# JitongZ/shockwave-replication

Hardware: AMD Instinct MI355X
Metric: Shockwave plan solves/sec at 900 jobs x 30 rounds (higher is better)
Workload: dtype f64 objective / fp32 ranking keys

## Files before the change

shockwave-replication_amd/csrc/sw_api.hip:

```cpp
#include <hip/hip_runtime.h>
#include <stdint.h>
#include <string.h>

#include <stdlib.h>

#include <algorithm>
#include <atomic>
#include <climits>
#include <new>
#include <string>
#include <thread>
#include <vector>

#include "../../include/shockwave_amd.h"
#include "sw_arith.h"
#include "sw_device.h"
#include "sw_handle.h"
#include "sw_p2x.h"
#include "sw_validate.h"

static int fuse_max_count() {
    static const int v = [] {
        const char* e = getenv("SW_FUSE_MAX");
        return e ? atoi(e) : 256;
    }();
    return v;
}

static int split_min_count() {
    static const int v = [] {
        const char* e = getenv("SW_SPLIT_MIN");
        return e ? atoi(e) : 256;
    }();
    return v;
}


extern "C" size_t sw_plan_kernel_lds_bytes(int one);
extern "C" hipError_t sw_launch_plan(const sw_batch_dev* B, int KT, int one, size_t lds,
                                     hipStream_t stream);
extern "C" hipError_t sw_launch_split(sw_batch_dev* B, size_t p2x_lds, hipStream_t stream);
extern "C" hipError_t sw_launch_p2x(const sw_batch_dev* B, int maxN, int maxT, hipStream_t stream);
extern "C" size_t sw_p2x_kernel_lds_bytes(int maxN, int maxT);

namespace {

thread_local std::string g_create_error;

}

namespace {
// ... 102 lines not shown
    }
    h->ev_pool.assign(2 * kEventPairs, nullptr);
    h->ev_p2x.assign(2 * kEventPairs, nullptr);
    for (size_t i = 0; e == hipSuccess && i < h->ev_pool.size(); ++i) e = hipEventCreate(&h->ev_pool[i]);
    for (size_t i = 0; e == hipSuccess && i < h->ev_p2x.size(); ++i) e = hipEventCreate(&h->ev_p2x[i]);
    if (e != hipSuccess) {
        g_create_error = std::string("HIP init failed: ") + hipGetErrorString(e);
        sw_destroy(h);
        return nullptr;
    }
    if (cfg && cfg->max_instances > 0 && cfg->max_total_jobs > 0) {
        size_t J = (size_t)cfg->max_total_jobs, I = (size_t)cfg->max_instances;
        if (h->d_in.reserve(in_block_bytes((int32_t)I, (int64_t)J)) ||
            h->d_res.reserve(res_block_bytes((int32_t)I, (int64_t)J, (int64_t)J * SW_MAX_ROUNDS)) ||
            h->d_masks.reserve(J) || h->d_nb.reserve(J) || h->d_lvl.reserve(I) ||
            h->d_p2ws.reserve(J * SW_P2X_ARR_BYTES) ||
            h->h_in.reserve(in_block_bytes((int32_t)I, (int64_t)J)) ||
            h->h_res.reserve(res_block_bytes((int32_t)I, (int64_t)J, (int64_t)J * SW_MAX_ROUNDS)) ||
            h->h_masks.reserve(J)) {
            g_create_error = "device reservation failed";
            sw_destroy(h);
            return nullptr;
        }
    }
    return h;
}

void sw_destroy(sw_handle* h) {
    if (!h) return;
    (void)hipSetDevice(h->device);
    if (h->stream) (void)hipStreamSynchronize(h->stream);
    if (h->up) (void)hipStreamSynchronize(h->up);
    if (h->dn) (void)hipStreamSynchronize(h->dn);
    sw_shard_release(h);
    sw_mmf_release(h);
    h->d_in.release(); h->d_res.release();
    h->d_ws_u8.release(); h->d_ws_u64.release(); h->d_ws_sort.release();
    h->d_ws_keys.release(); h->d_ws_jc.release(); h->d_stamps.release();
    h->d_masks.release(); h->d_p2ws.release(); h->d_nb.release(); h->d_lvl.release();
    h->h_in.release(); h->h_res.release();
    h->h_masks.release();
    for (hipEvent_t ev : h->ev_chunk)
        if (ev) (void)hipEventDestroy(ev);
    if (h->up) (void)hipStreamDestroy(h->up);
    if (h->dn) (void)hipStreamDestroy(h->dn);
    for (hipEvent_t ev : h->ev_xs)
        if (ev) (void)hipEventDestroy(ev);
    for (hipStream_t x : h->xs)
        if (x) (void)hipStreamDestroy(x);
    for (hipEvent_t ev : h->ev_pool)
        if (ev) (void)hipEventDestroy(ev);
    for (hipEvent_t ev : h->ev_p2x)
        if (ev) (void)hipEventDestroy(ev);
    if (h->own_stream && h->stream) (void)hipStreamDestroy(h->stream);
// ... 67 lines not shown
        P += (int64_t)pr.num_jobs * pr.future_rounds;
        maxN = std::max(maxN, pr.num_jobs);
        maxT = std::max(maxT, pr.future_rounds);
    }
    SW_HIP(h, hipStreamSynchronize(h->stream));
    if (h->up) SW_HIP(h, hipStreamSynchronize(h->up));
    if (h->dn) SW_HIP(h, hipStreamSynchronize(h->dn));
    if (collect_timing(h) != SW_OK) return SW_ERR_HIP;
    h->loaded = false;
    h->count = 0;
    h->total_jobs = 0;
    h->total_plan = 0;
    const size_t Jz = (size_t)std::max<int64_t>(J, 1);
    const size_t inb = in_block_bytes(std::max(count, 1), (int64_t)Jz), resb = res_block_bytes(std::max(count, 1), (int64_t)Jz, std::max<int64_t>(P, 1));
    if (h->d_in.reserve(inb) || h->d_res.reserve(resb) ||
        h->d_masks.reserve(Jz) || h->d_nb.reserve(Jz) || h->d_lvl.reserve(std::max(count, 1)))
        return fail(h, SW_ERR_HIP, "device allocation failed");
    if (maxN > SW_LDS_JOBS || maxT > 32) {
        const int KT = maxT <= 32 ? 32 : 64;
        if (h->d_ws_u8.reserve(Jz * SW_WS_U8) || h->d_ws_u64.reserve(Jz * SW_WS_U64 + (size_t)SW_WS_PAD_U64 * std::max(count, 1)) ||
            h->d_ws_sort.reserve(Jz * 4) || h->d_ws_keys.reserve(Jz * KT) ||
            h->d_ws_jc.reserve(Jz))
            return fail(h, SW_ERR_HIP, "workspace allocation failed");
    }
    if (h->d_p2ws.reserve(Jz * SW_P2X_ARR_BYTES))
        return fail(h, SW_ERR_HIP, "P2 exchange workspace allocation failed");
    if (h->h_in.reserve(inb) || h->h_res.reserve(resb) || h->h_masks.reserve(Jz))
        return fail(h, SW_ERR_HIP, "pinned allocation failed");
    set_views(h, std::max(count, 1), (int64_t)Jz, std::max<int64_t>(P, 1));
    h->inst.resize(count);
    h->Ns.resize(count);
// ... 109 lines not shown
    B.inst = h->d_inst + lo;
    B.count = hi - lo;
    B.KT = h->maxT <= 32 ? 32 : 64;
    B.w = h->d_w;
    B.d = h->d_d;
    B.F = h->d_F;
    B.E = h->d_E;
    B.R = h->d_R;
    B.p = h->d_p;
    B.plan = h->d_plan;
    B.planned = h->d_planned;
    B.masks = h->d_masks.p;
    B.out = h->d_out + lo;
    B.nb = h->d_nb.p;
    B.lvl = h->d_lvl.p + lo;
#ifdef SW_STAMPS
    B.stamps = h->d_stamps.p + (size_t)lo * SW_STAMP_SLOTS;
#endif
    const int one = h->maxN <= SW_LDS_JOBS && h->maxT <= 32;
    if (!one) {
        B.ws.u8 = h->d_ws_u8.p;
        B.ws.u64 = h->d_ws_u64.p;
        B.ws.sort = h->d_ws_sort.p;
        B.ws.keys = h->d_ws_keys.p;
        B.ws.jc = h->d_ws_jc.p;
    }
    B.p2ws = h->d_p2ws.p;
    size_t lds = sw_plan_kernel_lds_bytes(one);
    if (timed) {
        if (h->ev_used == kEventPairs && collect_timing(h) != SW_OK) return SW_ERR_HIP;
        SW_HIP(h, hipEventRecord(h->ev_pool[2 * h->ev_used], s));
    }
#ifdef SW_STAMPS
    const bool split = false;
#else
    const bool split = one && (force_split >= 0 ? force_split != 0 : B.count > split_min_count());
#endif
    B.fuse_p2x = one && (split || B.count <= fuse_max_count());
    if (B.fuse_p2x) lds = std::max(lds, sw_p2x_kernel_lds_bytes(h->maxN, h->maxT));
    hipError_t e = split ? sw_launch_split(&B, sw_p2x_kernel_lds_bytes(h->maxN, h->maxT), s)
                         : sw_launch_plan(&B, B.KT, one, lds, s);
    if (e != hipSuccess) return hip_fail(h, e, "plan kernel launch");
    if (timed) {
        SW_HIP(h, hipEventRecord(h->ev_pool[2 * h->ev_used + 1], s));
        SW_HIP(h, hipEventRecord(h->ev_p2x[2 * h->ev_used], s));
    }
    if (!B.fuse_p2x) {
        e = sw_launch_p2x(&B, h->maxN, h->maxT, s);
        if (e != hipSuccess) return hip_fail(h, e, "sw_p2x_kernel launch");
    }
    if (timed) {
        SW_HIP(h, hipEventRecord(h->ev_p2x[2 * h->ev_used + 1], s));
        h->ev_used++;
// ... 120 lines not shown
    static const int req = [] {
        const char* e = getenv("SW_RUN_STREAMS");
        return e ? atoi(e) : -1;
    }();
#ifdef SW_STAMPS
    return 1;
#endif
    const bool one = h->maxN <= SW_LDS_JOBS && h->maxT <= 32;
    if (!one || h->count <= split_min_count()) return 1;
    int ns = req >= 0 ? req : (h->count <= 2048 ? 2 : 1);
    ns = std::max(1, std::min(ns, kMaxRunStreams));
    return std::min(ns, std::max(1, h->count / 64));
}

int launch_streams(sw_handle* h, int ns) {
    if (h->xs.empty()) {
        h->xs.assign(kMaxRunStreams - 1, nullptr);
        h->ev_xs.assign(kMaxRunStreams, nullptr);
        for (auto& x : h->xs) SW_HIP(h, hipStreamCreateWithFlags(&x, hipStreamNonBlocking));
        for (auto& ev : h->ev_xs) SW_HIP(h, hipEventCreateWithFlags(&ev, hipEventDisableTiming));
    }
    const bool timed = h->timing;
    if (timed) {
        if (h->ev_used == kEventPairs && collect_timing(h) != SW_OK) return SW_ERR_HIP;
        SW_HIP(h, hipEventRecord(h->ev_pool[2 * h->ev_used], h->stream));
    }
    SW_HIP(h, hipEventRecord(h->ev_xs[0], h->stream));
    for (int c = 1; c < ns; ++c) SW_HIP(h, hipStreamWaitEvent(h->xs[c - 1], h->ev_xs[0], 0));
    int err = SW_OK;
    for (int c = 0; c < ns && err == SW_OK; ++c) {
        const int32_t lo = (int32_t)((int64_t)h->count * c / ns), hi = (int32_t)((int64_t)h->count * (c + 1) / ns);
        err = launch(h, lo, hi, c == 0 ? h->stream : h->xs[c - 1], false, h->keep_masks, 1);
    }
    for (int c = 1; c < ns; ++c) {
        SW_HIP(h, hipEventRecord(h->ev_xs[c], h->xs[c - 1]));
// ... 130 lines not shown
```

shockwave-replication_amd/csrc/sw_device.h:

```cpp
#pragma once
#include <stdint.h>

#include "sw_arith.h"

#define SW_STAMP_SLOTS 64
#define SW_LDS_JOBS 1024

struct sw_inst_dev {
    int32_t N, T, G, nb;
    int64_t job_off;
    int64_t plan_off;
    double delta, k;
    double beta[SW_BMAX];
    double ell[SW_BMAX];
};

struct sw_out_dev {
    double objective, utility, makespan, p2_objective, bound;
    int32_t iters, status;
};

struct sw_ws_dev {
    uint8_t* u8;
    uint64_t* u64;
// ... 21 lines not shown
    const int32_t* E;
    const double* R;
    const double* p;
    uint8_t* plan;
    int32_t* planned;
    uint64_t* masks;
    sw_out_dev* out;
    uint8_t* nb;
    sw_lvl_dev* lvl;
    int32_t only_slow;
    sw_ws_dev ws;
    unsigned char* p2ws;
    int32_t fuse_p2x;
    int32_t want_masks;
    int32_t lds_bytes;
    uint64_t* stamps;
};
```

shockwave-replication_amd/csrc/sw_handle.h:

```cpp
#pragma once
#include <hip/hip_runtime.h>
#include <stdint.h>

#include <algorithm>
#include <string>
#include <vector>

#include "../../include/shockwave_amd.h"
#include "sw_device.h"

struct sw_shard_state;

template <typename T>
struct DevBuf {
    T* p = nullptr;
    size_t cap = 0;
    hipError_t reserve(size_t n) {
        if (n <= cap) return hipSuccess;
        if (p) (void)hipFree(p);
        p = nullptr;
        cap = 0;
        size_t want = std::max<size_t>(n, 1);
        hipError_t e = hipMalloc((void**)&p, want * sizeof(T));
        if (e == hipSuccess) cap = want;
// ... 43 lines not shown
    std::vector<int32_t> Ns, Ts;
    sw_inst_dev* d_inst = nullptr;
    DevBuf<unsigned char> d_in, d_res;
    int32_t *d_w = nullptr, *d_F = nullptr, *d_E = nullptr, *d_planned = nullptr;
    double *d_d = nullptr, *d_R = nullptr, *d_p = nullptr;
    uint8_t* d_plan = nullptr;
    sw_out_dev* d_out = nullptr;
    size_t in_bytes = 0, res_bytes = 0;
    DevBuf<uint8_t> d_ws_u8;
    DevBuf<uint64_t> d_ws_u64, d_ws_sort;
    DevBuf<float> d_ws_keys;
    DevBuf<sw_jobc> d_ws_jc;
    DevBuf<uint64_t> d_masks;
    DevBuf<uint8_t> d_nb;
    DevBuf<sw_lvl_dev> d_lvl;
    DevBuf<unsigned char> d_p2ws;
    DevBuf<uint64_t> d_stamps;
    HostBuf<unsigned char> h_in, h_res;
    int32_t *h_w = nullptr, *h_F = nullptr, *h_E = nullptr, *h_planned = nullptr;
    double *h_d = nullptr, *h_R = nullptr, *h_p = nullptr;
    uint8_t* h_plan = nullptr;
    sw_out_dev* h_out = nullptr;
    HostBuf<uint64_t> h_masks;
    sw_inst_dev* h_inst = nullptr;
    hipStream_t up = nullptr, dn = nullptr;
    std::vector<hipEvent_t> ev_chunk;
    std::vector<hipStream_t> xs;
    std::vector<hipEvent_t> ev_xs;
    int32_t pend_count = 0;
    int64_t pend_jobs = 0, pend_plan = 0;
// ... 14 lines not shown
```

shockwave-replication_amd/csrc/sw_kernels.hip:

```cpp
#include <hip/hip_runtime.h>
#include <stdint.h>

#include "../../include/shockwave_amd.h"
#include "sw_arith.h"
#include "sw_block.h"
#include "sw_device.h"
#include "sw_pack.h"
#include "sw_bnb.h"
#include "sw_repair.h"
#include "sw_reround_dev.h"
#include "sw_p2x_inst.h"

namespace {

#ifdef SW_STAMPS
#define SW_STAMP(slot)                                                            \
    do {                                                                          \
        __syncthreads();                                                          \
        if (threadIdx.x == 0 && B.stamps) {                                       \
            uint64_t now_ = __builtin_amdgcn_s_memtime();                         \
            B.stamps[(size_t)inst_ * SW_STAMP_SLOTS + (slot)] += now_ - stamp_prev_;      \
            stamp_prev_ = now_;                                                   \
        }                                                                         \
    } while (0)
// ... 76 lines not shown
    double inv_delta;
    int64_t passes;
    double lsU, lsM;
    const sw_inst_dev* inst;
    const double* beta;
    const double* ell;
    const double* slope;
    sw_blk blk;
    const int32_t* w_in;
    const double* p_in;
#ifdef SW_STAMPS
    uint64_t* swp;
    uint64_t* lsp;
    uint64_t ls_t;
    uint64_t lsa[9];
#endif
    uint8_t *ncur, *lcur, *tkcur, *nbest, *placed, *placed2, *nfin;
    uint8_t* tiecur;
    uint64_t *ycur, *ybest, *y2;
    uint32_t* pst;
    uint64_t* pmask;
    int32_t* pord;
    uint64_t* sbuf;
    int32_t *H, *SH;
    sw_pack_lds* PL;
    int32_t pwc;
    int32_t* caps;
    int64_t* misc;
    sw_repair_t* rep;
    sw_bnb_ivl* bnb;
// ... 770 lines not shown
                k2 = 0;
            } else if (MODE != 2 && MODE != 5) {
                const double lvl = gval(j, s, nj - 1);
                const bool crit = k > 0.0 && lvl > Mb;
                k1 = crit ? (SW_CRIT_BIT | sw_bits(lvl)) : (MODE == 3 ? (uint64_t)jc(j, s).w : 0);
                k2 = kbits(j, s, nj - 1);
            } else {
                k1 = sw_ratio_key(p_in[j] / (double)nj);
                k2 = 0;
            }
            khi = k1;
            klo = ((uint64_t)k2 << 32) | (uint64_t)(0xFFFFFFFFu - (uint32_t)j);
        }
    }

    __device__ __forceinline__ void pack(int MODE, const uint8_t* nin, uint64_t* y,
                                         uint8_t* placed_out) {
        __syncthreads();
#ifdef SW_STAMPS
        uint64_t pk0_ = __builtin_amdgcn_s_memtime();
#define PK_STAMP(k)                                                      \
    do {                                                                 \
        const uint64_t n_ = __builtin_amdgcn_s_memtime();                \
        if (threadIdx.x == 0 && swp) swp[40 + (k)] += n_ - pk0_;         \
        pk0_ = n_;                                                       \
    } while (0)
#else
#define PK_STAMP(k) \
    do {            \
    } while (0)
#endif
        double Mb = 0.0;
        const int32_t* capsp = MODE == 5 ? caps : nullptr;
        if (MODE == 1 || MODE == 3) {
            for_jobs([&](int j, int s) { Mb = sw_max(Mb, gval(j, s, nin[j])); });
            Mb = blk.dmax(Mb);
        }
        int64_t act_l = 0;
        if constexpr (ONE) {
            constexpr int E = SW_JPT;
            uint64_t khi[E], klo[E];
#pragma unroll
            for (int s = 0; s < E; ++s) { khi[s] = 0; klo[s] = 0; }
            for_jobs([&](int j, int s) {
                key_of(MODE, nin, Mb, j, s, khi[s], klo[s]);
                act_l += nin_of(MODE, nin, j) > 0;
                if (owns(MODE, nin, j)) y[j] = 0;
            });
            int32_t A32;
            const int32_t abase = blk.exscan((int32_t)act_l, A32);
            const int A_ = A32;
            PK_STAMP(0);
#ifdef SW_STAMPS
            const uint64_t srt0_ = __builtin_amdgcn_s_memtime();
#endif
            const bool ratio = MODE == 2 || MODE == 4 || MODE == 5;
            if (ratio) {
#pragma unroll
                for (int s = 0; s < E; ++s)
                    khi[s] = khi[s] != 0 || klo[s] != 0
                                 ? (khi[s] << 11) | (uint64_t)(2047u - (0xFFFFFFFFu - (uint32_t)klo[s]))
                                 : 0ull;
            }
            if (SMALL || A_ <= SW_BLOCK) {
                uint64_t* xh = sbuf;
                uint64_t* xl = sbuf + SW_BLOCK;
                int b = abase;
#pragma unroll
                for (int s = 0; s < E; ++s)
                    if (klo[s] != 0) {
                        xh[b] = khi[s];
                        if constexpr (!SMALL) xl[b] = klo[s];
                        ++b;
                    }
                __syncthreads();
                const bool mine = (int)threadIdx.x < A_;
                uint64_t h1 = mine ? xh[threadIdx.x] : 0ull;
                uint64_t l1 = 0ull;
                if constexpr (SMALL) {
                    sort_one<false>(h1, l1, sbuf + SW_BLOCK);
                } else {
                    l1 = mine ? xl[threadIdx.x] : 0ull;
                    if (ratio) sort_one<false>(h1, l1, sbuf + 2 * SW_BLOCK);
                    else sort_one<true>(h1, l1, sbuf + 2 * SW_BLOCK);
                }
#ifdef SW_STAMPS
                if (threadIdx.x == 0 && swp) swp[7] += __builtin_amdgcn_s_memtime() - srt0_;
                pk0_ = __builtin_amdgcn_s_memtime();
#endif
                const int jp1 = !mine ? 0
                                : ratio ? (int)(2047u - (uint32_t)(h1 & 2047u))
                                        : (int)(0xFFFFFFFFu - (uint32_t)(l1 & 0xFFFFFFFFu));
                const uint32_t wq = MODE == 5 ? 1u : (uint32_t)w_in[jp1];
                uint32_t st1[1] = {mine ? ((uint32_t)nin[jp1] | (wq << 8)) : 0u};
                uint64_t mk1[1] = {0ull};
                PK_STAMP(1);
#ifdef SW_STAMPS
                sw_pack_rounds_one<SMALL>(PL, A_, T, G, st1[0], mk1[0], sbuf, capsp, swp);
#else
                sw_pack_rounds_one<SMALL>(PL, A_, T, G, st1[0], mk1[0], sbuf, capsp);
#endif
                PK_STAMP(2);
                for_jobs([&](int j, int s) {
                    (void)s;
                    if (owns(MODE, nin, j)) placed_out[j] = 0;
                });
                __syncthreads();
                if (mine) {
                    y[jp1] = mk1[0];
                    placed_out[jp1] = (uint8_t)(nin[jp1] - st_r(st1[0]));
                }
                __syncthreads();
                PK_STAMP(3);
            } else {
                if constexpr (!SMALL) {
                if (ratio) sort_regs64(khi);
                else sort_regs(khi, klo);
#ifdef SW_STAMPS
                if (threadIdx.x == 0 && swp) swp[7] += __builtin_amdgcn_s_memtime() - srt0_;
#endif
                uint32_t st[E];
                uint64_t mk[E];
                int jp[E];
#pragma unroll
                for (int s = 0; s < E; ++s) {
                    const int p = E * (int)threadIdx.x + s;
                    mk[s] = 0;
                    jp[s] = ratio ? (int)(2047u - (uint32_t)(khi[s] & 2047u))
                                  : (int)(0xFFFFFFFFu - (uint32_t)(klo[s] & 0xFFFFFFFFu));
                    const uint32_t wq = MODE == 5 ? 1u : (uint32_t)w_in[jp[s]];
                    st[s] = (p < A_) ? ((uint32_t)nin[jp[s]] | (wq << 8)) : 0u;
                }
#ifdef SW_STAMPS
                sw_pack_rounds<SW_JPT>(blk, PL, A_, T, G, st, mk, capsp, swp);
// ... 5 lines not shown
                    if (owns(MODE, nin, j)) placed_out[j] = 0;
                });
                __syncthreads();
#pragma unroll
                for (int s = 0; s < E; ++s) {
                    const int p = E * (int)threadIdx.x + s;
                    if (p < A_) {
                        y[jp[s]] = mk[s];
                        placed_out[jp[s]] = (uint8_t)(nin[jp[s]] - st_r(st[s]));
                    }
                }
                __syncthreads();
                            }
            }
        } else {
            int NPg = 1;
            while (NPg < N) NPg <<= 1;
            uint64_t* shi = sbuf;
            uint64_t* slo = sbuf + NPg;
            for (int i = threadIdx.x; i < NPg; i += SW_BLOCK) { shi[i] = 0; slo[i] = 0; }
            __syncthreads();
            for (int j = jlo(); j < jhi(); ++j) {
                uint64_t khi, klo;
                key_of(MODE, nin, Mb, j, 0, khi, klo);
                shi[j] = khi;
                slo[j] = klo;
                act_l += nin_of(MODE, nin, j) > 0;
                if (owns(MODE, nin, j)) y[j] = 0;
            }
            const int A_ = (int)blk.sum(act_l);
// ... 8 lines not shown
            }
            __syncthreads();
            if (wave_id() == 0) rounds(A_, PPL, capsp);
            __syncthreads();
            for (int j = jlo(); j < jhi(); ++j)
                if (owns(MODE, nin, j)) placed_out[j] = 0;
            __syncthreads();
            for (int p = threadIdx.x; p < A_; p += SW_BLOCK) {
                const int s = tslot(p, PPL);
                const int j = pord[s];
                y[j] = pmask[s];
                placed_out[j] = (uint8_t)(nin[j] - st_r(pst[s]));
            }
            __syncthreads();
        }
#undef PK_STAMP
    }

    __device__ __forceinline__ bool repair_pack(const uint8_t* nin, const uint64_t* yd,
                                                const uint8_t* pd, uint64_t* yout, uint8_t* pout) {
        sw_repair_t* R = rep;
        uint32_t* wset = reinterpret_cast<uint32_t*>(misc);
        int32_t* flag = reinterpret_cast<int32_t*>(misc) + 8;
        __syncthreads();
        for (int i = threadIdx.x; i < (int)(sizeof(sw_repair_t) / 4); i += SW_BLOCK)
            reinterpret_cast<int32_t*>(R)[i] = 0;
        if (threadIdx.x < 8) wset[threadIdx.x] = 0;
        __syncthreads();
        for_jobs([&](int j, int s) {
            (void)s;
            if (nin[j] > 0) atomicOr(&wset[(w_in[j] >> 5) & 7], 1u << (w_in[j] & 31));
        });
// ... 230 lines not shown
    if (one) {
        const size_t NJ = SW_LDS_JOBS;
        s += 8 * r16(NJ) + 3 * r16(8 * NJ) + r16(8 * 4 * SW_JPT * SW_BLOCK) + SW_JOB_LDS_BYTES;
    } else {
        s += 2 * r16(8 * (SW_RR_CAPMAX + 1)) + r16(8 * SW_RR_WORDS);
    }
    return s;
}

__host__ __device__ constexpr size_t sw_level_lds_bytes() {
    auto r16 = [](size_t b) { return (b + 15) & ~(size_t)15; };
    return r16(sizeof(sw_xchg)) + r16(sizeof(double) * 3 * SW_BMAX) +
           r16(sizeof(float) * SW_JPT * SW_SETUP_CH * SW_BLOCK) + SW_JOB_LDS_BYTES;
}

__host__ __device__ constexpr size_t sw_pack_lds_bytes() {
    auto r16 = [](size_t b) { return (b + 15) & ~(size_t)15; };
    const size_t NJ = SW_LDS_JOBS;
    return r16(sizeof(sw_xchg)) + r16(sizeof(sw_pack_lds)) + r16(sizeof(int64_t) * 8) +
           r16(sizeof(sw_repair_t)) + 3 * r16(NJ) + 2 * r16(8 * NJ) + r16(8 * 3 * SW_BLOCK);
}

template <int KT>
__device__ __forceinline__ void level_instance(const sw_batch_dev& B, unsigned char* smem, int inst_) {
    const sw_inst_dev* I = &B.inst[inst_];
    Ctx<KT, true> c;
    c.inst = I;
    c.N = I->N;
    c.T = I->T;
    c.G = I->G;
    c.nb = I->nb;
    c.C = (int64_t)I->G * I->T;
    c.k = I->k;
    c.inv_delta = 1.0 / I->delta;
    c.passes = 0;
// ... 92 lines not shown
        uint64_t m = ym[j];
        uint32_t wv[4] = {0u, 0u, 0u, 0u};
#pragma unroll
        for (int k = 0; k < 16; ++k) {
            wv[k >> 2] |= (uint32_t)((m >> t) & 1ull) << ((k & 3) * 8);
            if (++t == T) {
                t = 0;
                ++j;
                if (k < 15 && j < N) m = ym[j];
            }
        }
        dst[ci] = make_uint4(wv[0], wv[1], wv[2], wv[3]);
    }
}

__device__ __forceinline__ const uint64_t* pack_instance(const sw_batch_dev& B, unsigned char* smem, int inst_) {
    const sw_inst_dev* I = &B.inst[inst_];
    Ctx<32, true, true> c;
    c.inst = I;
    c.N = I->N;
    c.T = I->T;
    c.G = I->G;
    c.nb = I->nb;
    c.C = (int64_t)I->G * I->T;
    c.k = I->k;
    c.inv_delta = 1.0 / I->delta;
    const sw_lvl_dev lv = B.lvl[inst_];
    c.passes = lv.passes;
    c.q = (c.N + SW_BLOCK - 1) / SW_BLOCK;
    const int64_t jo = I->job_off;
    c.w_in = B.w + jo;
    c.p_in = B.p + jo;
#ifdef SW_STAMPS
    c.swp = nullptr;
    c.lsp = nullptr;
#endif
    size_t off = 0;
    auto carve = [&](size_t bytes) {
        unsigned char* p = smem + off;
        off += (bytes + 15) & ~(size_t)15;
        return p;
    };
    c.blk.X = (sw_xchg*)carve(sizeof(sw_xchg));
    c.blk.par = 0;
    c.beta = c.ell = c.slope = nullptr;
    c.PL = (sw_pack_lds*)carve(sizeof(sw_pack_lds));
    c.H = c.PL->H[0];
    c.SH = c.PL->SH[0];
    c.caps = c.PL->H[1];
    c.pwc = 0;
    c.misc = (int64_t*)carve(sizeof(int64_t) * 8);
    c.rep = (sw_repair_t*)carve(sizeof(sw_repair_t));
    const int NJ = SW_LDS_JOBS;
    c.nbest = carve(NJ);
    c.placed = carve(NJ);
    c.placed2 = carve(NJ);
    c.ncur = c.lcur = c.tkcur = c.nfin = c.tiecur = nullptr;
    c.bnb = nullptr;
    c.ycur = (uint64_t*)carve(sizeof(uint64_t) * NJ);
    c.y2 = (uint64_t*)carve(sizeof(uint64_t) * NJ);
    c.ybest = nullptr;
    c.sbuf = (uint64_t*)carve(sizeof(uint64_t) * 3 * SW_BLOCK);
    c.pst = nullptr;
    c.pord = nullptr;
    c.pmask = nullptr;
    c.gkeys = nullptr;
    c.gjc = nullptr;
    if (off != sw_pack_lds_bytes()) __builtin_trap();
    int64_t act_l = 0;
    c.for_jobs([&](int j, int s) {
        (void)s;
        c.nbest[j] = B.nb[jo + j];
        act_l += c.nbest[j] > 0;
    });
    sw_out_dev* out = &B.out[inst_];
    if (c.blk.sum(act_l) > SW_BLOCK) {
        if (threadIdx.x == 0) out->status = SW_STATUS_SLOW_MARK;
        return nullptr;
    }
    c.pack(4, c.nbest, c.ycur, c.placed);
    int64_t def_l = 0;
    c.for_jobs([&](int j, int s) {
        (void)s;
        def_l += (int64_t)c.w_in[j] * (c.nbest[j] - c.placed[j]);
    });
    int64_t dfc = c.blk.sum(def_l);
    c.passes++;
    int32_t status = 0;
    if (dfc != 0 && c.repair_pack(c.nbest, c.ycur, c.placed, c.y2, c.placed2)) {
        c.for_jobs([&](int j, int s) {
            (void)s;
            c.ycur[j] = c.y2[j];
        });
        c.passes++;
        dfc = 0;
// ... 44 lines not shown
                                          int inst) {
    const sw_inst_dev* I = &B.inst[inst];
    sw_out_dev* out = &B.out[inst];
    const int N = I->N, T = I->T, G = I->G;
    const int64_t jo = I->job_off;
    const int q = (N + SW_BLOCK - 1) / SW_BLOCK;
    const int j0 = sw_tid_opaque() * q, j1 = min(j0 + q, N);
    __syncthreads();
    int act = 0;
#pragma unroll
    for (int k = 0; k < 2; ++k) act += (j0 + k < j1 && ym[j0 + k] != 0ull) ? 1 : 0;
    const bool run = B.fuse_p2x && !(out->status & SW_STATUS_P2_FALLBACK);
    sw_p2x_lds* L = reinterpret_cast<sw_p2x_lds*>(smem);
    const size_t Lsz = (sizeof(sw_p2x_lds) + 15) & ~(size_t)15;
    unsigned char* var = smem + Lsz;
    sw_blk blk;
    blk.X = &L->X;
    blk.par = 0;
    int A = 0;
    const int a0 = blk.exscan(act, A);
    A = __builtin_amdgcn_readfirstlane(A);
    const uint64_t* yemit = ym;
    if (run && A > 0 && A <= SW_P2X_AMAX) {
        const size_t vb = (sw_p2x_var_bytes(A, T) + 15) & ~(size_t)15;
        const bool onchip = Lsz + vb + (size_t)SW_P2X_ARR_BYTES * A <= (size_t)B.lds_bytes &&
                            var + vb >= reinterpret_cast<const unsigned char*>(ym + N);
        unsigned char* base = onchip ? var + vb : B.p2ws + (size_t)SW_P2X_ARR_BYTES * jo;
        const size_t n = onchip ? (size_t)A : (size_t)N;
        sw_p2x_arrays X;
        X.cc = reinterpret_cast<double*>(base);
// ... 598 lines not shown
        if (B.fuse_p2x) {
            __syncthreads();
            sw_p2x_instance(B, B.p2ws, sw_smem, blockIdx.x);
        }
    }
}

template <int KT>
__global__ __launch_bounds__(SW_BLOCK, 4) void sw_level_kernel(sw_batch_dev B) {
    extern __shared__ __attribute__((aligned(16))) unsigned char sw_smem[];
    level_instance<KT>(B, sw_smem, blockIdx.x);
}

__global__ __launch_bounds__(SW_BLOCK, 8) void sw_pack_kernel(sw_batch_dev B) {
    extern __shared__ __attribute__((aligned(16))) unsigned char sw_smem[];
    const uint64_t* ym = pack_instance(B, sw_smem, blockIdx.x);
    if (ym) pack_tail(B, ym, sw_smem, blockIdx.x);
}

extern "C" size_t sw_plan_kernel_lds_bytes(int one) { return sw_plan_lds_bytes(one != 0); }

extern "C" hipError_t sw_launch_split(sw_batch_dev* B, size_t p2x_lds, hipStream_t stream) {
    dim3 grid(B->count), block(SW_BLOCK);
    B->only_slow = 0;
    B->fuse_p2x = 1;
    hipLaunchKernelGGL((sw_level_kernel<32>), grid, block, sw_level_lds_bytes(), stream, *B);
    B->lds_bytes = (int32_t)std::max(sw_pack_lds_bytes(), p2x_lds);
    hipLaunchKernelGGL(sw_pack_kernel, grid, block, (size_t)B->lds_bytes, stream, *B);
    B->only_slow = 1;
    hipLaunchKernelGGL((sw_plan_kernel<32, true>), grid, block, std::max(sw_plan_lds_bytes(true), p2x_lds),
                       stream, *B);
    B->only_slow = 0;
    return hipGetLastError();
}

extern "C" hipError_t sw_launch_plan(const sw_batch_dev* B, int KT, int one, size_t lds,
                                     hipStream_t stream) {
    dim3 grid(B->count), block(SW_BLOCK);
    if (KT == 32) {
        if (one) hipLaunchKernelGGL((sw_plan_kernel<32, true>), grid, block, lds, stream, *B);
        else hipLaunchKernelGGL((sw_plan_kernel<32, false>), grid, block, lds, stream, *B);
    } else {
        hipLaunchKernelGGL((sw_plan_kernel<64, false>), grid, block, lds, stream, *B);
// ... 4 lines not shown
```

Measured before the change: 2.549 million.

## Split pack stage into sort, wave-per-instance rounds, and place kernels

For large split batches (count at or above SW_LOOP_MIN, default 4096), the fused pack kernel is broken into three launches. A sort kernel writes ranked job words to global workspace. A rounds kernel runs the round-packing loop with one wave per instance, four instances per block. A place kernel reads the results back and runs the pack tail. The aim is to stop a whole block waiting on the serial rounds loop, at the cost of extra launches and global round-trips. Stream and event creation in launch_streams also becomes lazy, sized to the requested count.

Result: faster. 2.768 million, median of 6 (+8.6%).

```diff
diff --git a/shockwave-replication_amd/csrc/sw_api.hip b/shockwave-replication_amd/csrc/sw_api.hip
--- a/shockwave-replication_amd/csrc/sw_api.hip
+++ b/shockwave-replication_amd/csrc/sw_api.hip
@@ -35,6 +35,13 @@
     return v;
 }
 
+static int loop_min_count() {
+    static const int v = [] {
+        const char* e = getenv("SW_LOOP_MIN");
+        return e ? atoi(e) : 4096;
+    }();
+    return v;
+}
 
 extern "C" size_t sw_plan_kernel_lds_bytes(int one);
 extern "C" hipError_t sw_launch_plan(const sw_batch_dev* B, int KT, int one, size_t lds,
@@ -167,6 +174,7 @@
         if (h->d_in.reserve(in_block_bytes((int32_t)I, (int64_t)J)) ||
             h->d_res.reserve(res_block_bytes((int32_t)I, (int64_t)J, (int64_t)J * SW_MAX_ROUNDS)) ||
             h->d_masks.reserve(J) || h->d_nb.reserve(J) || h->d_lvl.reserve(I) ||
+            h->d_lws.reserve(J) || h->d_lwm.reserve(J) || h->d_lwa.reserve(I) ||
             h->d_p2ws.reserve(J * SW_P2X_ARR_BYTES) ||
             h->h_in.reserve(in_block_bytes((int32_t)I, (int64_t)J)) ||
             h->h_res.reserve(res_block_bytes((int32_t)I, (int64_t)J, (int64_t)J * SW_MAX_ROUNDS)) ||
@@ -191,6 +199,7 @@
     h->d_ws_u8.release(); h->d_ws_u64.release(); h->d_ws_sort.release();
     h->d_ws_keys.release(); h->d_ws_jc.release(); h->d_stamps.release();
     h->d_masks.release(); h->d_p2ws.release(); h->d_nb.release(); h->d_lvl.release();
+    h->d_lws.release(); h->d_lwm.release(); h->d_lwa.release();
     h->h_in.release(); h->h_res.release();
     h->h_masks.release();
     for (hipEvent_t ev : h->ev_chunk)
@@ -288,7 +297,8 @@
     const size_t Jz = (size_t)std::max<int64_t>(J, 1);
     const size_t inb = in_block_bytes(std::max(count, 1), (int64_t)Jz), resb = res_block_bytes(std::max(count, 1), (int64_t)Jz, std::max<int64_t>(P, 1));
     if (h->d_in.reserve(inb) || h->d_res.reserve(resb) ||
-        h->d_masks.reserve(Jz) || h->d_nb.reserve(Jz) || h->d_lvl.reserve(std::max(count, 1)))
+        h->d_masks.reserve(Jz) || h->d_nb.reserve(Jz) || h->d_lvl.reserve(std::max(count, 1)) ||
+        h->d_lws.reserve(Jz) || h->d_lwm.reserve(Jz) || h->d_lwa.reserve(std::max(count, 1)))
         return fail(h, SW_ERR_HIP, "device allocation failed");
     if (maxN > SW_LDS_JOBS || maxT > 32) {
         const int KT = maxT <= 32 ? 32 : 64;
@@ -428,6 +438,9 @@
     B.out = h->d_out + lo;
     B.nb = h->d_nb.p;
     B.lvl = h->d_lvl.p + lo;
+    B.lws = h->d_lws.p;
+    B.lwm = h->d_lwm.p;
+    B.lwa = h->d_lwa.p + lo;
 #ifdef SW_STAMPS
     B.stamps = h->d_stamps.p + (size_t)lo * SW_STAMP_SLOTS;
 #endif
@@ -451,6 +464,7 @@
     const bool split = one && (force_split >= 0 ? force_split != 0 : B.count > split_min_count());
 #endif
     B.fuse_p2x = one && (split || B.count <= fuse_max_count());
+    B.loop_split = split && B.count >= loop_min_count();
     if (B.fuse_p2x) lds = std::max(lds, sw_p2x_kernel_lds_bytes(h->maxN, h->maxT));
     hipError_t e = split ? sw_launch_split(&B, sw_p2x_kernel_lds_bytes(h->maxN, h->maxT), s)
                          : sw_launch_plan(&B, B.KT, one, lds, s);
@@ -601,11 +615,15 @@
 }
 
 int launch_streams(sw_handle* h, int ns) {
-    if (h->xs.empty()) {
-        h->xs.assign(kMaxRunStreams - 1, nullptr);
-        h->ev_xs.assign(kMaxRunStreams, nullptr);
-        for (auto& x : h->xs) SW_HIP(h, hipStreamCreateWithFlags(&x, hipStreamNonBlocking));
-        for (auto& ev : h->ev_xs) SW_HIP(h, hipEventCreateWithFlags(&ev, hipEventDisableTiming));
+    while ((int)h->xs.size() < ns - 1) {
+        hipStream_t x = nullptr;
+        SW_HIP(h, hipStreamCreateWithFlags(&x, hipStreamNonBlocking));
+        h->xs.push_back(x);
+    }
+    while ((int)h->ev_xs.size() < ns) {
+        hipEvent_t ev = nullptr;
+        SW_HIP(h, hipEventCreateWithFlags(&ev, hipEventDisableTiming));
+        h->ev_xs.push_back(ev);
     }
     const bool timed = h->timing;
     if (timed) {
diff --git a/shockwave-replication_amd/csrc/sw_device.h b/shockwave-replication_amd/csrc/sw_device.h
--- a/shockwave-replication_amd/csrc/sw_device.h
+++ b/shockwave-replication_amd/csrc/sw_device.h
@@ -59,5 +59,9 @@
     int32_t fuse_p2x;
     int32_t want_masks;
     int32_t lds_bytes;
+    int32_t loop_split;
+    uint32_t* lws;
+    uint64_t* lwm;
+    int32_t* lwa;
     uint64_t* stamps;
 };
diff --git a/shockwave-replication_amd/csrc/sw_handle.h b/shockwave-replication_amd/csrc/sw_handle.h
--- a/shockwave-replication_amd/csrc/sw_handle.h
+++ b/shockwave-replication_amd/csrc/sw_handle.h
@@ -81,6 +81,9 @@
     DevBuf<uint64_t> d_masks;
     DevBuf<uint8_t> d_nb;
     DevBuf<sw_lvl_dev> d_lvl;
+    DevBuf<uint32_t> d_lws;
+    DevBuf<uint64_t> d_lwm;
+    DevBuf<int32_t> d_lwa;
     DevBuf<unsigned char> d_p2ws;
     DevBuf<uint64_t> d_stamps;
     HostBuf<unsigned char> h_in, h_res;
diff --git a/shockwave-replication_amd/csrc/sw_kernels.hip b/shockwave-replication_amd/csrc/sw_kernels.hip
--- a/shockwave-replication_amd/csrc/sw_kernels.hip
+++ b/shockwave-replication_amd/csrc/sw_kernels.hip
@@ -114,6 +114,7 @@
     uint64_t* lsp;
     uint64_t ls_t;
     uint64_t lsa[9];
+    uint64_t pk0_, srt0;
 #endif
     uint8_t *ncur, *lcur, *tkcur, *nbest, *placed, *placed2, *nfin;
     uint8_t* tiecur;
@@ -914,11 +915,7 @@
         }
     }
 
-    __device__ __forceinline__ void pack(int MODE, const uint8_t* nin, uint64_t* y,
-                                         uint8_t* placed_out) {
-        __syncthreads();
 #ifdef SW_STAMPS
-        uint64_t pk0_ = __builtin_amdgcn_s_memtime();
 #define PK_STAMP(k)                                                      \
     do {                                                                 \
         const uint64_t n_ = __builtin_amdgcn_s_memtime();                \
@@ -930,94 +927,127 @@
     do {            \
     } while (0)
 #endif
+
+    template <bool ZY = true>
+    __device__ __forceinline__ bool pack_front(int MODE, const uint8_t* nin, uint64_t* y,
+                                               uint64_t (&khi)[SW_JPT], uint64_t (&klo)[SW_JPT], int& A_,
+                                               bool& mine, int& jp1, uint32_t& st1) {
+        constexpr int E = SW_JPT;
         double Mb = 0.0;
-        const int32_t* capsp = MODE == 5 ? caps : nullptr;
         if (MODE == 1 || MODE == 3) {
             for_jobs([&](int j, int s) { Mb = sw_max(Mb, gval(j, s, nin[j])); });
             Mb = blk.dmax(Mb);
         }
         int64_t act_l = 0;
+#pragma unroll
+        for (int s = 0; s < E; ++s) { khi[s] = 0; klo[s] = 0; }
+        for_jobs([&](int j, int s) {
+            key_of(MODE, nin, Mb, j, s, khi[s], klo[s]);
+            act_l += nin_of(MODE, nin, j) > 0;
+            if constexpr (ZY)
+                if (owns(MODE, nin, j)) y[j] = 0;
+        });
+        int32_t A32;
+        const int32_t abase = blk.exscan((int32_t)act_l, A32);
+        A_ = A32;
+        PK_STAMP(0);
+#ifdef SW_STAMPS
+        const uint64_t srt0_ = __builtin_amdgcn_s_memtime();
+        srt0 = srt0_;
+#endif
+        const bool ratio = MODE == 2 || MODE == 4 || MODE == 5;
+        if (ratio) {
+#pragma unroll
+            for (int s = 0; s < E; ++s)
+                khi[s] = khi[s] != 0 || klo[s] != 0
+                             ? (khi[s] << 11) | (uint64_t)(2047u - (0xFFFFFFFFu - (uint32_t)klo[s]))
+                             : 0ull;
+        }
+        if (!(SMALL || A_ <= SW_BLOCK)) return false;
+        uint64_t* xh = sbuf;
+        uint64_t* xl = sbuf + SW_BLOCK;
+        int b = abase;
+#pragma unroll
+        for (int s = 0; s < E; ++s)
+            if (klo[s] != 0) {
+                xh[b] = khi[s];
+                if constexpr (!SMALL) xl[b] = klo[s];
+                ++b;
+            }
+        __syncthreads();
+        mine = (int)threadIdx.x < A_;
+        uint64_t h1 = mine ? xh[threadIdx.x] : 0ull;
+        uint64_t l1 = 0ull;
+        if constexpr (SMALL) {
+            sort_one<false>(h1, l1, sbuf + SW_BLOCK);
+        } else {
+            l1 = mine ? xl[threadIdx.x] : 0ull;
+            if (ratio) sort_one<false>(h1, l1, sbuf + 2 * SW_BLOCK);
+            else sort_one<true>(h1, l1, sbuf + 2 * SW_BLOCK);
+        }
+#ifdef SW_STAMPS
+        if (threadIdx.x == 0 && swp) swp[7] += __builtin_amdgcn_s_memtime() - srt0_;
+        pk0_ = __builtin_amdgcn_s_memtime();
+#endif
+        jp1 = !mine ? 0
+              : ratio ? (int)(2047u - (uint32_t)(h1 & 2047u))
+                      : (int)(0xFFFFFFFFu - (uint32_t)(l1 & 0xFFFFFFFFu));
+        const uint32_t wq = MODE == 5 ? 1u : (uint32_t)w_in[jp1];
+        st1 = mine ? ((uint32_t)nin[jp1] | (wq << 8)) : 0u;
+        PK_STAMP(1);
+        return true;
+    }
+
+    __device__ __forceinline__ void pack_loop(int MODE, int A_, uint32_t& st1, uint64_t& mk1) {
+        const int32_t* capsp = MODE == 5 ? caps : nullptr;
+#ifdef SW_STAMPS
+        sw_pack_rounds_one<SMALL>(PL, A_, T, G, st1, mk1, sbuf, capsp, swp);
+#else
+        sw_pack_rounds_one<SMALL>(PL, A_, T, G, st1, mk1, sbuf, capsp);
+#endif
+        PK_STAMP(2);
+    }
+
+    __device__ __forceinline__ void pack_back(int MODE, const uint8_t* nin, uint64_t* y,
+                                              uint8_t* placed_out, bool mine, int jp1, uint32_t st1,
+                                              uint64_t mk1) {
+        for_jobs([&](int j, int s) {
+            (void)s;
+            if (owns(MODE, nin, j)) placed_out[j] = 0;
+        });
+        __syncthreads();
+        if (mine) {
+            y[jp1] = mk1;
+            placed_out[jp1] = (uint8_t)(nin[jp1] - st_r(st1));
+        }
+        __syncthreads();
+        PK_STAMP(3);
+    }
+
+    __device__ __forceinline__ void pack(int MODE, const uint8_t* nin, uint64_t* y,
+                                         uint8_t* placed_out) {
+        __syncthreads();
+#ifdef SW_STAMPS
+        pk0_ = __builtin_amdgcn_s_memtime();
+#endif
+        const int32_t* capsp = MODE == 5 ? caps : nullptr;
         if constexpr (ONE) {
             constexpr int E = SW_JPT;
             uint64_t khi[E], klo[E];
-#pragma unroll
-            for (int s = 0; s < E; ++s) { khi[s] = 0; klo[s] = 0; }
-            for_jobs([&](int j, int s) {
-                key_of(MODE, nin, Mb, j, s, khi[s], klo[s]);
-                act_l += nin_of(MODE, nin, j) > 0;
-                if (owns(MODE, nin, j)) y[j] = 0;
-            });
-            int32_t A32;
-            const int32_t abase = blk.exscan((int32_t)act_l, A32);
-            const int A_ = A32;
-            PK_STAMP(0);
-#ifdef SW_STAMPS
-            const uint64_t srt0_ = __builtin_amdgcn_s_memtime();
-#endif
-            const bool ratio = MODE == 2 || MODE == 4 || MODE == 5;
-            if (ratio) {
-#pragma unroll
-                for (int s = 0; s < E; ++s)
-                    khi[s] = khi[s] != 0 || klo[s] != 0
-                                 ? (khi[s] << 11) | (uint64_t)(2047u - (0xFFFFFFFFu - (uint32_t)klo[s]))
-                                 : 0ull;
-            }
-            if (SMALL || A_ <= SW_BLOCK) {
-                uint64_t* xh = sbuf;
-                uint64_t* xl = sbuf + SW_BLOCK;
-                int b = abase;
-#pragma unroll
-                for (int s = 0; s < E; ++s)
-                    if (klo[s] != 0) {
-                        xh[b] = khi[s];
-                        if constexpr (!SMALL) xl[b] = klo[s];
-                        ++b;
-                    }
-                __syncthreads();
-                const bool mine = (int)threadIdx.x < A_;
-                uint64_t h1 = mine ? xh[threadIdx.x] : 0ull;
-                uint64_t l1 = 0ull;
-                if constexpr (SMALL) {
-                    sort_one<false>(h1, l1, sbuf + SW_BLOCK);
-                } else {
-                    l1 = mine ? xl[threadIdx.x] : 0ull;
-                    if (ratio) sort_one<false>(h1, l1, sbuf + 2 * SW_BLOCK);
-                    else sort_one<true>(h1, l1, sbuf + 2 * SW_BLOCK);
-                }
-#ifdef SW_STAMPS
-                if (threadIdx.x == 0 && swp) swp[7] += __builtin_amdgcn_s_memtime() - srt0_;
-                pk0_ = __builtin_amdgcn_s_memtime();
-#endif
-                const int jp1 = !mine ? 0
-                                : ratio ? (int)(2047u - (uint32_t)(h1 & 2047u))
-                                        : (int)(0xFFFFFFFFu - (uint32_t)(l1 & 0xFFFFFFFFu));
-                const uint32_t wq = MODE == 5 ? 1u : (uint32_t)w_in[jp1];
-                uint32_t st1[1] = {mine ? ((uint32_t)nin[jp1] | (wq << 8)) : 0u};
-                uint64_t mk1[1] = {0ull};
-                PK_STAMP(1);
-#ifdef SW_STAMPS
-                sw_pack_rounds_one<SMALL>(PL, A_, T, G, st1[0], mk1[0], sbuf, capsp, swp);
-#else
-                sw_pack_rounds_one<SMALL>(PL, A_, T, G, st1[0], mk1[0], sbuf, capsp);
-#endif
-                PK_STAMP(2);
-                for_jobs([&](int j, int s) {
-                    (void)s;
-                    if (owns(MODE, nin, j)) placed_out[j] = 0;
-                });
-                __syncthreads();
-                if (mine) {
-                    y[jp1] = mk1[0];
-                    placed_out[jp1] = (uint8_t)(nin[jp1] - st_r(st1[0]));
-                }
-                __syncthreads();
-                PK_STAMP(3);
+            int A_, jp1 = 0;
+            bool mine = false;
+            uint32_t st1 = 0u;
+            if (pack_front(MODE, nin, y, khi, klo, A_, mine, jp1, st1)) {
+                uint64_t mk1 = 0ull;
+                pack_loop(MODE, A_, st1, mk1);
+                pack_back(MODE, nin, y, placed_out, mine, jp1, st1, mk1);
             } else {
                 if constexpr (!SMALL) {
+                const bool ratio = MODE == 2 || MODE == 4 || MODE == 5;
                 if (ratio) sort_regs64(khi);
                 else sort_regs(khi, klo);
 #ifdef SW_STAMPS
-                if (threadIdx.x == 0 && swp) swp[7] += __builtin_amdgcn_s_memtime() - srt0_;
+                if (threadIdx.x == 0 && swp) swp[7] += __builtin_amdgcn_s_memtime() - srt0;
 #endif
                 uint32_t st[E];
                 uint64_t mk[E];
@@ -1053,6 +1083,12 @@
                             }
             }
         } else {
+            double Mb = 0.0;
+            if (MODE == 1 || MODE == 3) {
+                for_jobs([&](int j, int s) { Mb = sw_max(Mb, gval(j, s, nin[j])); });
+                Mb = blk.dmax(Mb);
+            }
+            int64_t act_l = 0;
             int NPg = 1;
             while (NPg < N) NPg <<= 1;
             uint64_t* shi = sbuf;
@@ -1091,8 +1127,8 @@
             }
             __syncthreads();
         }
+    }
 #undef PK_STAMP
-    }
 
     __device__ __forceinline__ bool repair_pack(const uint8_t* nin, const uint64_t* yd,
                                                 const uint8_t* pd, uint64_t* yout, uint8_t* pout) {
@@ -1353,11 +1389,41 @@
            r16(sizeof(float) * SW_JPT * SW_SETUP_CH * SW_BLOCK) + SW_JOB_LDS_BYTES;
 }
 
-__host__ __device__ constexpr size_t sw_pack_lds_bytes() {
+struct sw_pack_carve {
+    size_t X, PL, misc, rep, nbest, placed, placed2, ycur, y2, sbuf, end;
+};
+__host__ __device__ constexpr sw_pack_carve sw_pack_offsets() {
     auto r16 = [](size_t b) { return (b + 15) & ~(size_t)15; };
     const size_t NJ = SW_LDS_JOBS;
-    return r16(sizeof(sw_xchg)) + r16(sizeof(sw_pack_lds)) + r16(sizeof(int64_t) * 8) +
-           r16(sizeof(sw_repair_t)) + 3 * r16(NJ) + 2 * r16(8 * NJ) + r16(8 * 3 * SW_BLOCK);
+    sw_pack_carve o{};
+    size_t off = 0;
+    o.X = off;       off += r16(sizeof(sw_xchg));
+    o.PL = off;      off += r16(sizeof(sw_pack_lds));
+    o.misc = off;    off += r16(sizeof(int64_t) * 8);
+    o.rep = off;     off += r16(sizeof(sw_repair_t));
+    o.nbest = off;   off += r16(NJ);
+    o.placed = off;  off += r16(NJ);
+    o.placed2 = off; off += r16(NJ);
+    o.ycur = off;    off += r16(8 * NJ);
+    o.y2 = off;      off += r16(8 * NJ);
+    o.sbuf = off;    off += r16(8 * 3 * SW_BLOCK);
+    o.end = off;
+    return o;
+}
+__host__ __device__ constexpr size_t sw_pack_lds_bytes() { return sw_pack_offsets().end; }
+
+struct sw_sort_carve {
+    size_t X, nbest, sbuf, end;
+};
+__host__ __device__ constexpr sw_sort_carve sw_sort_offsets() {
+    auto r16 = [](size_t b) { return (b + 15) & ~(size_t)15; };
+    sw_sort_carve o{};
+    size_t off = 0;
+    o.X = off;     off += r16(sizeof(sw_xchg));
+    o.nbest = off; off += r16((size_t)SW_LDS_JOBS);
+    o.sbuf = off;  off += r16(8 * 3 * SW_BLOCK);
+    o.end = off;
+    return o;
 }
 
 template <int KT>
@@ -1480,9 +1546,8 @@
     }
 }
 
-__device__ __forceinline__ const uint64_t* pack_instance(const sw_batch_dev& B, unsigned char* smem, int inst_) {
-    const sw_inst_dev* I = &B.inst[inst_];
-    Ctx<32, true, true> c;
+template <class CTX>
+__device__ __forceinline__ void pack_ctx_scalars(CTX& c, const sw_batch_dev& B, const sw_inst_dev* I) {
     c.inst = I;
     c.N = I->N;
     c.T = I->T;
@@ -1491,60 +1556,84 @@
     c.C = (int64_t)I->G * I->T;
     c.k = I->k;
     c.inv_delta = 1.0 / I->delta;
-    const sw_lvl_dev lv = B.lvl[inst_];
-    c.passes = lv.passes;
+    c.passes = 0;
     c.q = (c.N + SW_BLOCK - 1) / SW_BLOCK;
-    const int64_t jo = I->job_off;
-    c.w_in = B.w + jo;
-    c.p_in = B.p + jo;
+    c.w_in = B.w + I->job_off;
+    c.p_in = B.p + I->job_off;
 #ifdef SW_STAMPS
     c.swp = nullptr;
     c.lsp = nullptr;
 #endif
-    size_t off = 0;
-    auto carve = [&](size_t bytes) {
-        unsigned char* p = smem + off;
-        off += (bytes + 15) & ~(size_t)15;
-        return p;
-    };
-    c.blk.X = (sw_xchg*)carve(sizeof(sw_xchg));
     c.blk.par = 0;
     c.beta = c.ell = c.slope = nullptr;
-    c.PL = (sw_pack_lds*)carve(sizeof(sw_pack_lds));
-    c.H = c.PL->H[0];
-    c.SH = c.PL->SH[0];
-    c.caps = c.PL->H[1];
+    c.PL = nullptr;
+    c.H = c.SH = c.caps = nullptr;
     c.pwc = 0;
-    c.misc = (int64_t*)carve(sizeof(int64_t) * 8);
-    c.rep = (sw_repair_t*)carve(sizeof(sw_repair_t));
-    const int NJ = SW_LDS_JOBS;
-    c.nbest = carve(NJ);
-    c.placed = carve(NJ);
-    c.placed2 = carve(NJ);
+    c.misc = nullptr;
+    c.rep = nullptr;
+    c.nbest = c.placed = c.placed2 = nullptr;
     c.ncur = c.lcur = c.tkcur = c.nfin = c.tiecur = nullptr;
     c.bnb = nullptr;
-    c.ycur = (uint64_t*)carve(sizeof(uint64_t) * NJ);
-    c.y2 = (uint64_t*)carve(sizeof(uint64_t) * NJ);
-    c.ybest = nullptr;
-    c.sbuf = (uint64_t*)carve(sizeof(uint64_t) * 3 * SW_BLOCK);
+    c.ycur = c.y2 = c.ybest = nullptr;
+    c.sbuf = nullptr;
     c.pst = nullptr;
     c.pord = nullptr;
     c.pmask = nullptr;
     c.gkeys = nullptr;
     c.gjc = nullptr;
-    if (off != sw_pack_lds_bytes()) __builtin_trap();
-    int64_t act_l = 0;
-    c.for_jobs([&](int j, int s) {
-        (void)s;
-        c.nbest[j] = B.nb[jo + j];
-        act_l += c.nbest[j] > 0;
-    });
+}
+
+static_assert(SW_LDS_JOBS <= (1 << 11), "the job index fits the position word");
+#define SW_LWA_MARKED (-1)
+
+template <bool WS>
+__device__ __forceinline__ const uint64_t* pack_instance(const sw_batch_dev& B, unsigned char* smem, int inst_) {
+    const sw_inst_dev* I = &B.inst[inst_];
+    Ctx<32, true, true> c;
+    pack_ctx_scalars(c, B, I);
+    const sw_lvl_dev lv = B.lvl[inst_];
+    c.passes = lv.passes;
+    const int64_t jo = I->job_off;
+    constexpr sw_pack_carve O = sw_pack_offsets();
+    c.blk.X = (sw_xchg*)(smem + O.X);
+    c.PL = (sw_pack_lds*)(smem + O.PL);
+    c.H = c.PL->H[0];
+    c.SH = c.PL->SH[0];
+    c.caps = c.PL->H[1];
+    c.misc = (int64_t*)(smem + O.misc);
+    c.rep = (sw_repair_t*)(smem + O.rep);
+    c.nbest = smem + O.nbest;
+    c.placed = smem + O.placed;
+    c.placed2 = smem + O.placed2;
+    c.ycur = (uint64_t*)(smem + O.ycur);
+    c.y2 = (uint64_t*)(smem + O.y2);
+    c.sbuf = (uint64_t*)(smem + O.sbuf);
     sw_out_dev* out = &B.out[inst_];
-    if (c.blk.sum(act_l) > SW_BLOCK) {
-        if (threadIdx.x == 0) out->status = SW_STATUS_SLOW_MARK;
-        return nullptr;
-    }
-    c.pack(4, c.nbest, c.ycur, c.placed);
+    if constexpr (!WS) {
+        int64_t act_l = 0;
+        c.for_jobs([&](int j, int s) {
+            (void)s;
+            c.nbest[j] = B.nb[jo + j];
+            act_l += c.nbest[j] > 0;
+        });
+        if (c.blk.sum(act_l) > SW_BLOCK) {
+            if (threadIdx.x == 0) out->status = SW_STATUS_SLOW_MARK;
+            return nullptr;
+        }
+        c.pack(4, c.nbest, c.ycur, c.placed);
+    } else {
+        const int A_ = sw_u32(B.lwa[inst_]);
+        if (A_ == SW_LWA_MARKED) return nullptr;
+        c.for_jobs([&](int j, int s) {
+            (void)s;
+            c.nbest[j] = B.nb[jo + j];
+            c.ycur[j] = 0;
+        });
+        const bool mine = (int)threadIdx.x < A_;
+        const uint32_t word = mine ? B.lws[jo + threadIdx.x] : 0u;
+        const uint64_t mk1 = mine ? B.lwm[jo + threadIdx.x] : 0ull;
+        c.pack_back(4, c.nbest, c.ycur, c.placed, mine, (int)(word >> 16), word & 0xFFFFu, mk1);
+    }
     int64_t def_l = 0;
     c.for_jobs([&](int j, int s) {
         (void)s;
@@ -1619,6 +1708,8 @@
     sw_p2x_lds* L = reinterpret_cast<sw_p2x_lds*>(smem);
     const size_t Lsz = (sizeof(sw_p2x_lds) + 15) & ~(size_t)15;
     unsigned char* var = smem + Lsz;
+    static_assert(offsetof(sw_p2x_lds, X) + sizeof(sw_xchg) <= sw_pack_offsets().ycur,
+                  "the pack's masks lie past the exchange words of sw_p2x_lds");
     sw_blk blk;
     blk.X = &L->X;
     blk.par = 0;
@@ -2247,7 +2338,91 @@
 
 __global__ __launch_bounds__(SW_BLOCK, 8) void sw_pack_kernel(sw_batch_dev B) {
     extern __shared__ __attribute__((aligned(16))) unsigned char sw_smem[];
-    const uint64_t* ym = pack_instance(B, sw_smem, blockIdx.x);
+    const uint64_t* ym = pack_instance<false>(B, sw_smem, blockIdx.x);
+    if (ym) pack_tail(B, ym, sw_smem, blockIdx.x);
+}
+
+__global__ __launch_bounds__(SW_BLOCK, 8) void sw_sort_kernel(sw_batch_dev B) {
+    extern __shared__ __attribute__((aligned(16))) unsigned char sw_smem[];
+    const int inst_ = blockIdx.x;
+    const sw_inst_dev* I = &B.inst[inst_];
+    Ctx<32, true, true> c;
+    pack_ctx_scalars(c, B, I);
+    const int64_t jo = I->job_off;
+    constexpr sw_sort_carve O = sw_sort_offsets();
+    c.blk.X = (sw_xchg*)(sw_smem + O.X);
+    c.nbest = sw_smem + O.nbest;
+    c.sbuf = (uint64_t*)(sw_smem + O.sbuf);
+    int64_t act_l = 0;
+    c.for_jobs([&](int j, int s) {
+        (void)s;
+        c.nbest[j] = B.nb[jo + j];
+        act_l += c.nbest[j] > 0;
+    });
+    if (c.blk.sum(act_l) > SW_BLOCK) {
+        if (threadIdx.x == 0) {
+            B.out[inst_].status = SW_STATUS_SLOW_MARK;
+            B.lwa[inst_] = SW_LWA_MARKED;
+        }
+        return;
+    }
+    __syncthreads();
+    uint64_t khi[SW_JPT], klo[SW_JPT];
+    int A_, jp1 = 0;
+    bool mine = false;
+    uint32_t st1 = 0u;
+    c.template pack_front<false>(4, c.nbest, nullptr, khi, klo, A_, mine, jp1, st1);
+    if (mine) B.lws[jo + threadIdx.x] = st1 | ((uint32_t)jp1 << 16);
+    if (threadIdx.x == 0) B.lwa[inst_] = A_;
+}
+
+struct sw_rounds_lds {
+    sw_pack_lds L;
+    uint64_t mk[SW_BLOCK];
+};
+
+template <int E1>
+__device__ __forceinline__ void rounds_wave_ws(sw_rounds_lds* S, int A, int T, int G, uint32_t* ws,
+                                               uint64_t* wm) {
+    const int lane = lane_id();
+    uint32_t st[E1];
+#pragma unroll
+    for (int i = 0; i < E1; ++i) {
+        const int p = E1 * lane + i;
+        st[i] = p < A ? (ws[p] & 0xFFFFu) : 0u;
+    }
+    sw_pack_rounds_wave<E1>(&S->L, T, G, st, S->mk);
+#pragma unroll
+    for (int i = 0; i < E1; ++i) {
+        const int p = E1 * lane + i;
+        if (p < A) {
+            ws[p] = (ws[p] & 0xFFFF0000u) | st[i];
+            wm[p] = S->mk[p];
+        }
+    }
+}
+
+#define SW_LOOP_WPB 4
+__global__ __launch_bounds__(64 * SW_LOOP_WPB, 6) void sw_rounds_kernel(sw_batch_dev B) {
+    __shared__ __attribute__((aligned(16))) sw_rounds_lds S_[SW_LOOP_WPB];
+    const int inst_ = (int)blockIdx.x * SW_LOOP_WPB + wave_id();
+    if (inst_ >= B.count) return;
+    const int A = sw_u32(B.lwa[inst_]);
+    if (A <= 0) return;
+    const sw_inst_dev* I = &B.inst[inst_];
+    const int T = sw_u32(I->T), G = sw_u32(I->G);
+    uint32_t* ws = B.lws + I->job_off;
+    uint64_t* wm = B.lwm + I->job_off;
+    sw_rounds_lds* S = &S_[wave_id()];
+    if (A <= 128) rounds_wave_ws<2>(S, A, T, G, ws, wm);
+    else if (A <= 256) rounds_wave_ws<4>(S, A, T, G, ws, wm);
+    else if (A <= 384) rounds_wave_ws<6>(S, A, T, G, ws, wm);
+    else rounds_wave_ws<8>(S, A, T, G, ws, wm);
+}
+
+__global__ __launch_bounds__(SW_BLOCK, 8) void sw_place_kernel(sw_batch_dev B) {
+    extern __shared__ __attribute__((aligned(16))) unsigned char sw_smem[];
+    const uint64_t* ym = pack_instance<true>(B, sw_smem, blockIdx.x);
     if (ym) pack_tail(B, ym, sw_smem, blockIdx.x);
 }
 
@@ -2259,7 +2434,14 @@
     B->fuse_p2x = 1;
     hipLaunchKernelGGL((sw_level_kernel<32>), grid, block, sw_level_lds_bytes(), stream, *B);
     B->lds_bytes = (int32_t)std::max(sw_pack_lds_bytes(), p2x_lds);
-    hipLaunchKernelGGL(sw_pack_kernel, grid, block, (size_t)B->lds_bytes, stream, *B);
+    if (B->loop_split) {
+        hipLaunchKernelGGL(sw_sort_kernel, grid, block, sw_sort_offsets().end, stream, *B);
+        dim3 rgrid((B->count + SW_LOOP_WPB - 1) / SW_LOOP_WPB), rblock(64 * SW_LOOP_WPB);
+        hipLaunchKernelGGL(sw_rounds_kernel, rgrid, rblock, 0, stream, *B);
+        hipLaunchKernelGGL(sw_place_kernel, grid, block, (size_t)B->lds_bytes, stream, *B);
+    } else {
+        hipLaunchKernelGGL(sw_pack_kernel, grid, block, (size_t)B->lds_bytes, stream, *B);
+    }
     B->only_slow = 1;
     hipLaunchKernelGGL((sw_plan_kernel<32, true>), grid, block, std::max(sw_plan_lds_bytes(true), p2x_lds),
                        stream, *B);
```
